# hellojialee/OffsetGuided

Measured on NVIDIA B200. Metric: decoded images/s @640 long-edge, higher is better.
Workload: dtype f32

## Files before the change

include/og_decoder.h:

```cpp
#ifndef OG_DECODER_H_
#define OG_DECODER_H_

#include <stdint.h>

#ifdef __cplusplus
extern "C" {
#endif

#define OG_ABI_VERSION 2
#define OG_MAX_IN_FLIGHT 16
#define OG_LIMB_COLS 13
#define OG_POSE_COLS 6
#define OG_MAX_KEYPOINTS 64
#define OG_MAX_LIMBS 64
#define OG_MAX_TOPK 128
#define OG_DTYPE_F32 0
#define OG_DTYPE_BF16 1
#define OG_DTYPE_F16 2

typedef enum og_status {
    OG_OK = 0,
    OG_ERR_INVALID_ARGUMENT = 1,
    OG_ERR_CUDA = 2,
    OG_ERR_OUT_OF_MEMORY = 3,
// ... 129 lines not shown
int og_plan_launch(og_handle *h, int32_t plan_id, void *stream);

typedef struct og_result {
    const float *poses;
    const int32_t *offsets;
    const int32_t *counts;
    int32_t n_images;
    int32_t total_rows;
    int32_t n_keypoints;
    int32_t buffer_id;
    const float *coco_keypoints;
    const double *coco_scores;
    const int32_t *coco_images;
} og_result;
int og_fetch_result(og_handle *h, og_result *out);

int og_set_frames(og_handle *h, const double *frames_host, int n);
int og_fetch_poses(og_handle *h, const float **poses_host, const int32_t **offset_host,
                   const int32_t **count_host, int32_t *total_rows);
int og_pending(const og_handle *h);

int og_copy_intermediates(og_handle *h, int n, float *det_score_dev, int32_t *det_index_dev,
                          float *limbs_dev, void *stream);

int64_t og_launch_count(const og_handle *h);

int og_set_fused(og_handle *h, int enable);

int og_set_graph(og_handle *h, int enable);
int64_t og_graph_replay_count(const og_handle *h);
int64_t og_graph_build_count(const og_handle *h);

int og_debug_k3_profile(uint64_t *out16, int reset);
int64_t og_fused_redo_count(const og_handle *h);
int64_t og_k3_redo_count(const og_handle *h);

int og_set_zero_copy(og_handle *h, int enable);
int64_t og_zero_copy_count(const og_handle *h);

int og_enable_stage_timing(og_handle *h, int enable);
int og_last_stage_times_ms(og_handle *h, float *out6);

#ifdef __cplusplus
}
#endif
#endif
```

offsetguided_b200/_lib.py:

```python
import ctypes
import os

_PKG_DIR = os.path.dirname(os.path.abspath(__file__))
LIB_PATH = os.path.join(_PKG_DIR, 'libogdecoder.so')

OG_LIMB_COLS = 13
OG_POSE_COLS = 6
OG_MAX_TOPK = 128
OG_MAX_IN_FLIGHT = 16
OG_DTYPE_F32 = 0
OG_DTYPE_BF16 = 1
OG_DTYPE_F16 = 2

c_int32_p = ctypes.POINTER(ctypes.c_int32)
c_float_p = ctypes.POINTER(ctypes.c_float)


class OgConfig(ctypes.Structure):
    _fields_ = [
        ('n_keypoints', ctypes.c_int32),
        ('n_limbs', ctypes.c_int32),
        ('limb_from', c_int32_p),
        ('limb_to', c_int32_p),
        ('topk', ctypes.c_int32),
# ... 47 lines not shown
    'og_flip_fuse_f32': (_i, [_vp, _vp, _vp, c_int32_p, c_int32_p, c_int32_p, _i, _i, _i, _i, _vp, _vp, _vp]),
    'og_flip_average_f32': (_i, [_vp, c_int32_p, _i, _i, _i, _i, _i, _vp, _vp]),
    'og_flip_cat_offsets_f32': (_i, [_vp, c_int32_p, c_int32_p, _i, _i, _i, _i, _i, _vp, _vp]),
    'og_resize_f32': (_i, [_vp, _vp, _i, _i, _i, _i, _i, _vp]),
    'og_decode_maps': (_i, [_vp, _vp, _vp, _vp, _i, _i, _i, _vp]),
    'og_decode_maps_ex': (_i, [_vp, _vp, _vp, _vp, _vp, _i, _i, _i, _i, _i, _vp]),
    'og_decode_features_host': (_i, [_vp, _vp, _vp, _i, _i, _i, _i, _i, _i, _i,
                                     c_int32_p, c_int32_p, c_int32_p, _i, _vp]),
    'og_decode_features_dev': (_i, [_vp, _vp, _vp, _i, _i, _i, _i, _i, _i, _i,
                                    c_int32_p, c_int32_p, c_int32_p, _i, _vp]),
    'og_decode_features_dev_ex': (_i, [_vp, _vp, _vp, _i, ctypes.c_int64, ctypes.c_int64, _i, _i, _i, _i, _i,
                                       _i, _i, c_int32_p, c_int32_p, c_int32_p, _i, _vp]),
    'og_decode_features_dev_strided': (_i, [_vp, _vp, _vp, _i, _i64_p, _i64_p, _i, _i, _i, _i, _i, _i, _i,
                                            c_int32_p, c_int32_p, c_int32_p, _i, _vp]),
    'og_fetch_poses': (_i, [_vp, ctypes.POINTER(c_float_p), ctypes.POINTER(c_int32_p),
                            ctypes.POINTER(c_int32_p), ctypes.POINTER(ctypes.c_int32)]),
    'og_decode_features_heads_dev': (_i, [_vp, _vp, _vp, _vp, _vp, _i, _i, _i, _i, _i, _i, _i,
                                          _i, _i, c_int32_p, c_int32_p, c_int32_p, _i, _vp]),
    'og_plan_features': (_i, [_vp, _vp, _vp, _i, ctypes.c_int64, ctypes.c_int64, _i, _i, _i, _i, _i,
                              _i, _i, c_int32_p, c_int32_p, c_int32_p, _i, ctypes.POINTER(ctypes.c_int32)]),
    'og_plan_features_strided': (_i, [_vp, _vp, _vp, _i, _i64_p, _i64_p, _i, _i, _i, _i, _i, _i, _i,
                                      c_int32_p, c_int32_p, c_int32_p, _i, ctypes.POINTER(ctypes.c_int32)]),
    'og_plan_launch': (_i, [_vp, ctypes.c_int32, _vp]),
    'og_fetch_result': (_i, [_vp, ctypes.POINTER(OgResult)]),
    'og_set_frames': (_i, [_vp, ctypes.POINTER(ctypes.c_double), _i]),
    'og_pending': (_i, [_vp]),
    'og_copy_intermediates': (_i, [_vp, _i, _vp, _vp, _vp, _vp]),
    'og_launch_count': (ctypes.c_int64, [_vp]),
    'og_set_fused': (_i, [_vp, _i]),
    'og_set_graph': (_i, [_vp, _i]),
    'og_graph_replay_count': (ctypes.c_int64, [_vp]),
    'og_graph_build_count': (ctypes.c_int64, [_vp]),
    'og_debug_k3_profile': (_i, [ctypes.POINTER(ctypes.c_uint64), _i]),
    'og_fused_redo_count': (ctypes.c_int64, [_vp]),
    'og_k3_redo_count': (ctypes.c_int64, [_vp]),
    'og_set_zero_copy': (_i, [_vp, _i]),
    'og_zero_copy_count': (ctypes.c_int64, [_vp]),
    'og_enable_stage_timing': (_i, [_vp, _i]),
    'og_last_stage_times_ms': (_i, [_vp, c_float_p]),
}

_lib = None


def load():
    global _lib
    if _lib is not None:
        return _lib
    if not os.path.exists(LIB_PATH):
        raise OgError(
            f'{LIB_PATH} is missing: build it with `python -m offsetguided_b200.build` '
            '(or __graft_entry__.build()).  There is no CPU fallback.')
    lib = ctypes.CDLL(LIB_PATH)
    for name, (restype, argtypes) in SIGNATURES.items():
        fn = getattr(lib, name)
        fn.restype = restype
        fn.argtypes = argtypes
    if lib.og_abi_version() != 2:
        raise OgError(f'ABI version mismatch: library reports {lib.og_abi_version()}')
    _lib = lib
    return lib


def check(status):
    if status != 0:
        lib = load()
# ... 13 lines not shown
```

offsetguided_b200/csrc/og_api.cu:

```cuda
#include <math.h>
#include <stdlib.h>
#include <string.h>

#include <algorithm>
#include <new>
#include <vector>

#include "og_common.cuh"

namespace og {

static thread_local char g_error[1024] = "";

void set_error(const char *fmt, ...) {
    va_list ap;
    va_start(ap, fmt);
    vsnprintf(g_error, sizeof(g_error), fmt, ap);
    va_end(ap);
}

}

using namespace og;

// ... 1560 lines not shown
    return OG_OK;
}

int64_t og_zero_copy_count(const og_handle *h) { return h ? h->zero_copy_calls : 0; }

int og_set_frames(og_handle *h, const double *frames_host, int n) {
    OG_REQUIRE(h && n >= 0 && (n == 0 || frames_host), "og_set_frames: null pointer");
    for (int i = 0; i < n; ++i)
        OG_REQUIRE(frames_host[4 * i + 2] != 0.0 && frames_host[4 * i + 3] != 0.0,
                   "og_set_frames: image %d has a zero scale", i);
    if (n > h->staged_cap) {
        double *grown = static_cast<double *>(realloc(h->staged_frames, (size_t)(n + 8) * 4 * sizeof(double)));
        if (!grown) {
            set_error("host allocation failed");
            return OG_ERR_OUT_OF_MEMORY;
        }
        h->staged_frames = grown;
        h->staged_cap = n + 8;
    }
    if (n) memcpy(h->staged_frames, frames_host, (size_t)n * 4 * sizeof(double));
    h->staged_n = n;
    return OG_OK;
}

int og_set_graph(og_handle *h, int enable) {
    OG_REQUIRE(h, "og_set_graph: null handle");
    h->graph_enabled = enable != 0;
    return OG_OK;
}

int64_t og_graph_replay_count(const og_handle *h) { return h ? h->graph_replays : 0; }
int64_t og_graph_build_count(const og_handle *h) { return h ? h->graph_builds : 0; }

int og_debug_k3_profile(uint64_t *out16, int reset) {
    OG_REQUIRE(out16, "og_debug_k3_profile: null pointer");
    return read_k3_profile(reinterpret_cast<unsigned long long *>(out16), reset != 0);
}

int og_enable_stage_timing(og_handle *h, int enable) {
    OG_REQUIRE(h, "og_enable_stage_timing: null handle");
    OG_TRY(check_device(h));
    if (enable) {
        for (int i = 0; i < kSlots; ++i)
            for (int e = 0; e < kStageEvents; ++e)
                if (!h->slots[i].ev[e]) OG_CUDA_TRY(cudaEventCreate(&h->slots[i].ev[e]));
    }
    h->timing = enable != 0;
    return OG_OK;
}

int og_last_stage_times_ms(og_handle *h, float *out6) {
    OG_REQUIRE(h && out6, "og_last_stage_times_ms: null pointer");
    OG_REQUIRE(h->fetched_slot >= 0 && h->slots[h->fetched_slot].timed,
               "og_last_stage_times_ms: enable stage timing, decode and fetch first");
    ResultSlot *slot = &h->slots[h->fetched_slot];
    OG_CUDA_TRY(cudaEventSynchronize(slot->ev[kStageEvents - 1]));
    static const int first[6] = {0, 1, 3, 4, 5, 6};
    for (int i = 0; i < 6; ++i)
        OG_CUDA_TRY(cudaEventElapsedTime(&out6[i], slot->ev[first[i]], slot->ev[first[i] + 1]));
    return OG_OK;
}

}
```

offsetguided_b200/csrc/og_common.cuh:

```cuda
#pragma once

#include <cuda_bf16.h>
#include <cuda_fp16.h>
#include <cuda_runtime.h>
#include <stdint.h>
#include <stdio.h>
#include <stdarg.h>

#include "../../include/og_decoder.h"

namespace og {

void set_error(const char *fmt, ...);

#define OG_CUDA_TRY(expr)                                                          \
    do {                                                                           \
        cudaError_t err__ = (expr);                                                \
        if (err__ != cudaSuccess) {                                                \
            og::set_error("%s:%d: %s failed: %s", __FILE__, __LINE__, #expr,       \
                          cudaGetErrorString(err__));                              \
            return err__ == cudaErrorMemoryAllocation ? OG_ERR_OUT_OF_MEMORY       \
                                                       : OG_ERR_CUDA;              \
        }                                                                          \
    } while (0)

#define OG_REQUIRE(cond, ...)                                                      \
    do {                                                                           \
        if (!(cond)) {                                                             \
            og::set_error(__VA_ARGS__);                                            \
            return OG_ERR_INVALID_ARGUMENT;                                        \
        }                                                                          \
    } while (0)

#define OG_TRY(expr)                                                               \
    do {                                                                           \
        int st__ = (expr);                                                         \
        if (st__ != OG_OK) return st__;                                            \
    } while (0)

constexpr int kChainCarveoutPercent = 58;

#ifdef __CUDACC__
template <auto Kernel>
inline void prefer_chain_carveout() {
    static unsigned long long done = 0ull;
    int dev = 0;
    if (cudaGetDevice(&dev) != cudaSuccess || dev < 0 || dev >= 64) return;
    if ((done >> dev) & 1ull) return;
    if (cudaFuncSetAttribute(Kernel, cudaFuncAttributePreferredSharedMemoryCarveout, kChainCarveoutPercent) !=
        cudaSuccess)
        (void)cudaGetLastError();
    done |= 1ull << dev;
}
#endif

constexpr int kCandCap = 2048;

__device__ __forceinline__ uint32_t ordered_bits(float v) {
    uint32_t u = __float_as_uint(v);
    return (u & 0x80000000u) ? ~u : (u | 0x80000000u);
}
__device__ __forceinline__ float from_ordered_bits(uint32_t o) {
    uint32_t u = (o & 0x80000000u) ? (o & 0x7fffffffu) : ~o;
    return __uint_as_float(u);
}
__device__ __forceinline__ uint64_t make_key(float v, uint32_t idx) {
    return ((uint64_t)(~ordered_bits(v)) << 32) | idx;
}
__device__ __forceinline__ float key_value(uint64_t key) {
    return from_ordered_bits(~(uint32_t)(key >> 32));
}

struct SkeletonDev {
// ... 71 lines not shown
    HeadSource jitter_lr;
};

struct PrepOut {
    int32_t *prep;
    float4 *rec;
    int32_t *cnt;
    float dist_max;
    int use_scale;
    int32_t *clear_word;
};

int launch_limb_score(const float *det_score, const int32_t *det_index, const float *offs,
                      const OffsetSource *lowres, const FlipTablesDev *flips, const float *scales,
                      const LimbExtras *extras, int n, int c, int l, int k, int h, int w,
                      const SkeletonDev &sk, float thre_hmp, float min_len, float resize_factor,
                      float *out_limbs, const PrepOut *prep, cudaStream_t s);

struct ChannelPerm {
    int32_t src[128];
};
int launch_flip_average(const float *in2n, float *out, int n, int ch, int h, int w,
                        const ChannelPerm &perm, bool negate_even, cudaStream_t s);
int launch_flip_cat_offsets(const float *off2n, float *out, int n, int l, int h, int w,
                            const ChannelPerm &limb_flip, const ChannelPerm &reserved, cudaStream_t s);

bool fused_supported(int n, int c, int scale, int h, int w);
void fused_scratch(int n, int c, int h, int w, int scale, size_t *flag_bytes, size_t *list_ints);
int launch_fused_candidates(const MapView &hmp, const FlipTablesDev &flips, int n, int n_total, int c, int h, int w,
                            int scale, bool cubic, bool flip, float thre, uint32_t *cand_count,
                            uint64_t *cand_keys, uint8_t *block_flag, int32_t *block_list,
                            int32_t *n_active, float *nhwc_heat, int sm_count, bool clear_first,
                            cudaStream_t s, int64_t *launches);

int launch_fuse_planes(const MapView &hmp, const FlipTablesDev &flips, int n, int c, int h, int w, bool flip,
                       const int32_t *plane_list, int count, float *out, cudaStream_t s);

struct CocoOut {
    const double *frames;
    float *keypoints;
    double *scores;
    int32_t *images;
    int image0;
};

struct GroupLaunch {
    int n, c, l, k;
    SkeletonDev sk;
    float dist_max;
    int use_scale;
    double person_thre;
    int sort_dim;
    int warp_rows;
    float *slab;
    size_t slab_stride;
    int32_t *prep;
    float4 *rec;
    int32_t *cnt;
    int32_t *redo;
    CocoOut coco;
    int32_t *lazy_flag;
};
int read_k3_profile(unsigned long long *out16, bool reset);
size_t group_smem_bytes(const GroupLaunch &g);
size_t group_warp_smem_bytes(const GroupLaunch &g);
size_t group_prep_ints(const GroupLaunch &g);
// ... 20 lines not shown
```

offsetguided_b200/csrc/og_fused.cu:

```cuda
#include "og_common.cuh"
#include "og_interp.cuh"

#include <algorithm>

namespace og {

namespace {

#ifndef OG_K1F_MIN_CTAS
#define OG_K1F_MIN_CTAS 4
#endif
constexpr int kFusedThreads = 256;
constexpr int kScanThreads = 256;
constexpr int kBlockCellsH = 8;
constexpr int kSub = 4;
constexpr unsigned kFull = 0xffffffffu;

__device__ __forceinline__ float4 ldg_stream4(const float *p) {
    float4 v;
    asm volatile("ld.global.nc.L1::no_allocate.v4.f32 {%0, %1, %2, %3}, [%4];"
                 : "=f"(v.x), "=f"(v.y), "=f"(v.z), "=f"(v.w)
                 : "l"(p));
    return v;
}

__device__ __forceinline__ float4 load_cells4(const float *p) { return ldg_stream4(p); }
__device__ __forceinline__ float4 load_cells4(const __nv_bfloat16 *p) {
    unsigned lo, hi;
    asm volatile("ld.global.nc.L1::no_allocate.v2.u32 {%0, %1}, [%2];" : "=r"(lo), "=r"(hi) : "l"(p));
    return make_float4(__uint_as_float(lo << 16), __uint_as_float(lo & 0xffff0000u),
                       __uint_as_float(hi << 16), __uint_as_float(hi & 0xffff0000u));
}

__device__ __forceinline__ float4 load_cells4(const __half *p) {
    unsigned lo, hi;
    asm volatile("ld.global.nc.L1::no_allocate.v2.u32 {%0, %1}, [%2];" : "=r"(lo), "=r"(hi) : "l"(p));
    const float2 a = __half22float2(*reinterpret_cast<const __half2 *>(&lo));
    const float2 b = __half22float2(*reinterpret_cast<const __half2 *>(&hi));
    return make_float4(a.x, a.y, b.x, b.y);
}

__device__ __forceinline__ unsigned abs_bits(float v) { return __float_as_uint(fabsf(v)); }

template <typename T, bool kFlip, bool kVec>
__global__ void __launch_bounds__(kScanThreads)
amax_scan_kernel(const T *__restrict__ hmp, size_t img_stride, const FlipTablesDev ft,
                 int N, int C, int h, int w, int bw_shift, int halo, float limit,
                 uint8_t *__restrict__ block_flag, int plane0, int planes, int per_plane) {
    const unsigned idx = blockIdx.x * (unsigned)kScanThreads + threadIdx.x;
    const unsigned pl = idx / (unsigned)per_plane;
    if (pl >= (unsigned)planes) return;
    const int local = (int)(idx - pl * (unsigned)per_plane);
    const int sxs = (w + kSub - 1) / kSub;
    const int band = local / sxs, sx = local - band * sxs;
    const int y0 = band * 2 * kSub, x0 = sx * kSub;
    const int block_w = 1 << bw_shift;
    const int bxs = (w + block_w - 1) >> bw_shift, bys = (h + kBlockCellsH - 1) / kBlockCellsH;
    {
        const int plane = plane0 + (int)pl;
        const int n = plane / C, c = plane - n * C;
        const T *a = hmp + (size_t)n * img_stride + (size_t)c * h * w;
        const T *b = nullptr;
        if (kFlip) b = hmp + (size_t)(N + n) * img_stride + (size_t)ft.kp[c] * h * w;
        uint8_t *flags = block_flag + (size_t)plane * bys * bxs;
        auto flag_blocks = [&](int xa, int xb, int y) {
            const int bx_lo = max(xa - halo, 0) >> bw_shift, bx_hi = min((xb + halo) >> bw_shift, bxs - 1);
            const int by_lo = max(y - halo, 0) / kBlockCellsH, by_hi = min((y + halo) / kBlockCellsH, bys - 1);
            for (int by = by_lo; by <= by_hi; ++by)
                for (int bx = bx_lo; bx <= bx_hi; ++bx) flags[by * bxs + bx] = 1;
        };
        if (kVec) {
#pragma unroll 1
            for (int r0 = 0; r0 < 2 * kSub; r0 += kSub) {
                float4 va[kSub], vb[kSub];
#pragma unroll
                for (int r = 0; r < kSub; ++r) {
                    const int y = min(y0 + r0 + r, h - 1);
                    va[r] = load_cells4(a + (size_t)y * w + x0);
                    if (kFlip) vb[r] = load_cells4(b + (size_t)y * w + (w - kSub - x0));
                }
                auto fused_row = [&](int r) {
                    float4 f = va[r];
                    if (kFlip) {
                        f.x = __fmul_rn(__fadd_rn(f.x, vb[r].w), 0.5f);
                        f.y = __fmul_rn(__fadd_rn(f.y, vb[r].z), 0.5f);
                        f.z = __fmul_rn(__fadd_rn(f.z, vb[r].y), 0.5f);
                        f.w = __fmul_rn(__fadd_rn(f.w, vb[r].x), 0.5f);
                    }
                    return f;
                };
                unsigned hot = 0u;
#pragma unroll
                for (int r = 0; r < kSub; ++r) {
                    const float4 f = fused_row(r);
                    const unsigned q = max(max(abs_bits(f.x), abs_bits(f.y)), max(abs_bits(f.z), abs_bits(f.w)));
                    if (!(__uint_as_float(q) < limit) && y0 + r0 + r < h) hot |= 1u << r;
                }
                if (hot != 0u) {
#pragma unroll
                    for (int r = 0; r < kSub; ++r) {
                        if (!((hot >> r) & 1u)) continue;
                        const float4 f = fused_row(r);
                        const bool c0 = !(fabsf(f.x) < limit), c1 = !(fabsf(f.y) < limit), c2 = !(fabsf(f.z) < limit),
                                   c3 = !(fabsf(f.w) < limit);
                        const int first = c0 ? 0 : (c1 ? 1 : (c2 ? 2 : 3));
                        const int last = c3 ? 3 : (c2 ? 2 : (c1 ? 1 : 0));
                        flag_blocks(x0 + first, x0 + last, y0 + r0 + r);
                    }
                }
            }
        } else {
            for (int r = 0; r < 2 * kSub; ++r) {
                const int y = y0 + r;
                if (y >= h) break;
                for (int j = 0; j < kSub; ++j) {
                    const int x = x0 + j;
                    if (x >= w) break;
                    float v = load_cell(a + (size_t)y * w + x);
                    if (kFlip) v = __fmul_rn(__fadd_rn(v, load_cell(b + (size_t)y * w + (w - 1 - x))), 0.5f);
                    if (!(fabsf(v) < limit)) flag_blocks(x, x, y);
                }
            }
        }
    }
}

constexpr int kNhwcPixels = 32;
constexpr int kNhwcThreads = 256;

template <typename T, bool kFlip>
__global__ void __launch_bounds__(kNhwcThreads)
amax_scan_nhwc_kernel(const T *__restrict__ hmp, size_t img_stride, size_t pix_stride, const FlipTablesDev ft,
                      int N, int C, int h, int w, int bw_shift, int halo, float limit,
                      uint8_t *__restrict__ block_flag, float *__restrict__ out) {
    __shared__ float s_row[OG_MAX_KEYPOINTS][kNhwcPixels + 1];
    const int gxs = (w + kNhwcPixels - 1) / kNhwcPixels, bands = (h + kBlockCellsH - 1) / kBlockCellsH;
    const unsigned cta = blockIdx.x;
    const int gx = (int)(cta % (unsigned)gxs);
    const int band = (int)((cta / (unsigned)gxs) % (unsigned)bands);
    const int n = (int)(cta / ((unsigned)gxs * (unsigned)bands));
    const int x0 = gx * kNhwcPixels, y0 = band * kBlockCellsH;
    const int px_n = min(kNhwcPixels, w - x0), y_end = min(y0 + kBlockCellsH, h);
    const int block_w = 1 << bw_shift;
    const int bxs = (w + block_w - 1) >> bw_shift, bys = (h + kBlockCellsH - 1) / kBlockCellsH;
    const size_t hw = (size_t)h * w;
    const T *a = hmp + (size_t)n * img_stride;
    const T *b = kFlip ? hmp + (size_t)(N + n) * img_stride : nullptr;
    const int cells = px_n * C;
    for (int y = y0; y < y_end; ++y) {
        for (int i = threadIdx.x; i < cells; i += kNhwcThreads) {
            const int px = i / C, c = i - px * C;
            const int x = x0 + px;
            float v = load_cell(a + ((size_t)y * w + x) * pix_stride + c);
            if (kFlip)
// ... 220 lines not shown
            for (int p = 0; p < S; ++p) {
                const bool pass = (mask >> p) & 1u;
                if (!__any_sync(kFull, pass)) continue;
                const float vp = v[p], vc = v[p + 1], vn = v[p + 2];
                const float lp = __shfl_up_sync(kFull, vp, 1), lc = __shfl_up_sync(kFull, vc, 1),
                            ln = __shfl_up_sync(kFull, vn, 1);
                const float rp = __shfl_down_sync(kFull, vp, 1), rc = __shfl_down_sync(kFull, vc, 1),
                            rn = __shfl_down_sync(kFull, vn, 1);
                if (pass) {
                    const int Y = Y0 + q * S + p;
                    bool peak = true;
                    if (lane > 0) peak = peak && !(lp > vc) && !(lc > vc) && !(ln > vc);
                    if (lane < 31) peak = peak && !(rp > vc) && !(rc > vc) && !(rn > vc);
                    if (peak && ((lane == 0 && X0 > 0) || (lane == 31 && X + 1 < W))) {
                        const int Xn = lane == 0 ? X - 1 : X + 1;
                        for (int dy = -1; dy <= 1 && peak; ++dy) {
                            if (Y + dy < 0 || Y + dy >= H) continue;
                            peak = !(tile_value<S, kCubic, LW, HALO>(lo, cx0, cy0, Xn, Y + dy) > vc);
                        }
                    }
                    if (peak) {
                        const uint32_t pos = atomicAdd(&cand_count[plane], 1u);
                        if (pos < (uint32_t)kCandCap)
                            cand_keys[(size_t)plane * kCandCap + pos] =
                                make_key(vc + 0.0f, (uint32_t)(Y * W + X));
                    }
                }
            }
        }
    }
}

template <typename Kernel>
int resident_per_sm(Kernel kernel) {
    int per_sm = 1;
    if (cudaOccupancyMaxActiveBlocksPerMultiprocessor(&per_sm, kernel, kFusedThreads, 0) != cudaSuccess ||
        per_sm < 1)
        per_sm = 1;
    return per_sm;
}

constexpr int kCtaWaves = 4;

template <typename T, int S, bool kCubic, bool kFlip>
int launch_blocks_t(const T *hmp, size_t img_stride, int n_total, int h, int w, float thre,
                    const int4 *block_list, const int32_t *n_active, uint32_t *cand_count,
                    uint64_t *cand_keys, int sm_count, size_t blocks, cudaStream_t s) {
    auto kernel = fused_block_kernel<T, S, kCubic, kFlip>;
    static const int per_sm = resident_per_sm(kernel);
    const int grid = (int)std::min<size_t>((blocks + kFusedThreads / 32 - 1) / (kFusedThreads / 32),
                                           (size_t)sm_count * per_sm * kCtaWaves);
    prefer_chain_carveout<fused_block_kernel<T, S, kCubic, kFlip>>();
    kernel<<<grid, kFusedThreads, 0, s>>>(hmp, img_stride, n_total, h, w, thre, block_list, n_active,
                                          cand_count, cand_keys);
    OG_CUDA_TRY(cudaGetLastError());
    return OG_OK;
}

template <typename T, int S>
int launch_blocks_s(const T *hmp, size_t img_stride, int n_total, int h, int w, bool cubic, bool flip,
                    float thre, const int4 *block_list, const int32_t *n_active, uint32_t *cand_count,
                    uint64_t *cand_keys, int sm_count, size_t blocks, cudaStream_t s) {
    if (cubic)
        return flip ? launch_blocks_t<T, S, true, true>(hmp, img_stride, n_total, h, w, thre, block_list, n_active, cand_count, cand_keys, sm_count, blocks, s)
                    : launch_blocks_t<T, S, true, false>(hmp, img_stride, n_total, h, w, thre, block_list, n_active, cand_count, cand_keys, sm_count, blocks, s);
    return flip ? launch_blocks_t<T, S, false, true>(hmp, img_stride, n_total, h, w, thre, block_list, n_active, cand_count, cand_keys, sm_count, blocks, s)
                : launch_blocks_t<T, S, false, false>(hmp, img_stride, n_total, h, w, thre, block_list, n_active, cand_count, cand_keys, sm_count, blocks, s);
}

inline size_t block_count(int n, int c, int h, int w, int scale) {
    const int bw = 32 / scale;
    return (size_t)n * c * ((w + bw - 1) / bw) * ((h + kBlockCellsH - 1) / kBlockCellsH);
}

}

bool fused_supported(int n, int c, int scale, int h, int w) {
    if (!(scale == 2 || scale == 4 || scale == 8)) return false;
    return block_count(n, c, h, w, scale) < 0x1fffffffULL && h < 65536 * kBlockCellsH && w < 65536 &&
           (unsigned long long)h * scale * w * scale < 0xffffffffULL;
}

void fused_scratch(int n, int c, int h, int w, int scale, size_t *flag_bytes, size_t *list_ints) {
    *flag_bytes = block_count(n, c, h, w, scale);
    *list_ints = 4 * block_count(n, c, h, w, scale);
}

namespace {
inline int scan_bw_shift(int scale) { return scale == 2 ? 4 : (scale == 4 ? 3 : 2); }
inline int scan_halo(bool cubic) { return cubic ? 2 : 1; }
inline float scan_limit(float thre, bool cubic) { return thre / (cubic ? 1.95f : 1.001f); }

template <typename T>
int launch_scan_nhwc_t(const T *hmp, size_t img_stride, size_t pix_stride, const FlipTablesDev &kp_flip_dev, int n,
                       int n_total, int c, int h, int w, int scale, bool cubic, bool flip, float thre,
                       uint8_t *block_flag, float *out, cudaStream_t s) {
    const long long ctas = (long long)n * ((w + kNhwcPixels - 1) / kNhwcPixels) *
                           ((h + kBlockCellsH - 1) / kBlockCellsH);
    if (ctas > 0x7fffffffLL) {
        set_error("fused K1: %lld scan CTAs of channels-last maps exceed one launch", ctas);
        return OG_ERR_UNSUPPORTED;
    }
#define OG_SCAN_NHWC(FLIP)                                                                                      \
    (prefer_chain_carveout<amax_scan_nhwc_kernel<T, FLIP>>(),                                                    \
     amax_scan_nhwc_kernel<T, FLIP><<<(unsigned)ctas, kNhwcThreads, 0, s>>>(                                     \
         hmp, img_stride, pix_stride, kp_flip_dev, n_total, c, h, w, scan_bw_shift(scale), scan_halo(cubic),     \
         scan_limit(thre, cubic), block_flag, out))
    if (flip) OG_SCAN_NHWC(true); else OG_SCAN_NHWC(false);
#undef OG_SCAN_NHWC
    OG_CUDA_TRY(cudaGetLastError());
    return OG_OK;
}

template <typename T>
int launch_fused_t(const T *hmp, size_t img_stride, const FlipTablesDev &kp_flip_dev, int n, int n_total,
                   int c, int h, int w, int scale, bool cubic, bool flip, float thre,
                   uint32_t *cand_count, uint64_t *cand_keys, uint8_t *block_flag, int32_t *block_list,
                   int32_t *n_active, int sm_count, bool clear_first, bool scan, cudaStream_t s,
                   int64_t *launches) {
    if (clear_first) {
        OG_CUDA_TRY(cudaMemsetAsync(cand_count, 0, sizeof(uint32_t) * (size_t)n * c, s));
        OG_CUDA_TRY(cudaMemsetAsync(n_active, 0, sizeof(int32_t), s));
    }

    const int sxs = (w + kSub - 1) / kSub, bands = (h + 2 * kSub - 1) / (2 * kSub);
    const int per_plane = bands * sxs, planes = scan ? n * c : 0;
    const int planes_per_launch = std::max(1, (int)std::min<long long>(n * c, 0x7fffffffLL / per_plane - 1));
    const int block_w = 32 / scale, halo = scan_halo(cubic);
    const int bw_shift = scan_bw_shift(scale);
    const float limit = scan_limit(thre, cubic);
    const size_t vec_bytes = 4 * sizeof(T);
    const bool vec = (w % kSub) == 0 && (reinterpret_cast<uintptr_t>(hmp) % vec_bytes) == 0 &&
                     (img_stride * sizeof(T)) % vec_bytes == 0;
#define OG_SCAN(FLIP, VEC)                                                                                     \
    (prefer_chain_carveout<amax_scan_kernel<T, FLIP, VEC>>(),                                                  \
     amax_scan_kernel<T, FLIP, VEC><<<scan_grid, kScanThreads, 0, s>>>(hmp, img_stride, kp_flip_dev, n_total, c, h, \
                                                                      w, bw_shift, halo, limit, block_flag, p0, pn, \
                                                                      per_plane))
    for (int p0 = 0; p0 < planes; p0 += planes_per_launch) {
        const int pn = std::min(planes_per_launch, planes - p0);
        const unsigned scan_grid = (unsigned)(((long long)pn * per_plane + kScanThreads - 1) / kScanThreads);
        if (flip) {
            if (vec) OG_SCAN(true, true); else OG_SCAN(true, false);
        } else {
            if (vec) OG_SCAN(false, true); else OG_SCAN(false, false);
        }
    }
#undef OG_SCAN
    OG_CUDA_TRY(cudaGetLastError());

    const size_t blocks = block_count(n, c, h, w, scale);
    int4 *list4 = reinterpret_cast<int4 *>(block_list);
    prefer_chain_carveout<block_list_kernel>();
    block_list_kernel<<<(unsigned)((blocks + 255) / 256), 256, 0, s>>>(
        block_flag, kp_flip_dev, c, flip ? 1 : 0, (w + block_w - 1) / block_w,
        (h + kBlockCellsH - 1) / kBlockCellsH, (long long)blocks, list4, n_active);
    OG_CUDA_TRY(cudaGetLastError());

    int st;
    switch (scale) {
        case 2: st = launch_blocks_s<T, 2>(hmp, img_stride, n_total, h, w, cubic, flip, thre, list4, n_active, cand_count, cand_keys, sm_count, blocks, s); break;
        case 4: st = launch_blocks_s<T, 4>(hmp, img_stride, n_total, h, w, cubic, flip, thre, list4, n_active, cand_count, cand_keys, sm_count, blocks, s); break;
        default: st = launch_blocks_s<T, 8>(hmp, img_stride, n_total, h, w, cubic, flip, thre, list4, n_active, cand_count, cand_keys, sm_count, blocks, s); break;
    }
    if (st == OG_OK && launches) *launches += 3;
    return st;
}
}

int launch_fused_candidates(const MapView &hmp, const FlipTablesDev &kp_flip_dev, int n, int n_total, int c,
                            int h, int w, int scale, bool cubic, bool flip, float thre,
                            uint32_t *cand_count, uint64_t *cand_keys, uint8_t *block_flag,
                            int32_t *block_list, int32_t *n_active, float *nhwc_heat, int sm_count,
                            bool clear_first, cudaStream_t s, int64_t *launches) {
    if (n == 0) return OG_OK;
    if (!fused_supported(n, c, scale, h, w)) {
        set_error("fused K1: scale %d / %d x %d maps are outside the supported range", scale, h, w);
        return OG_ERR_UNSUPPORTED;
    }
    if (hmp.is_channels_last()) {
        if (clear_first) {
            OG_CUDA_TRY(cudaMemsetAsync(cand_count, 0, sizeof(uint32_t) * (size_t)n * c, s));
            OG_CUDA_TRY(cudaMemsetAsync(n_active, 0, sizeof(int32_t), s));
        }
        int st;
        if (hmp.dtype == OG_DTYPE_BF16)
            st = launch_scan_nhwc_t(static_cast<const __nv_bfloat16 *>(hmp.ptr), hmp.image_stride, hmp.pixel_stride,
                                    kp_flip_dev, n, n_total, c, h, w, scale, cubic, flip, thre, block_flag, nhwc_heat, s);
        else if (hmp.dtype == OG_DTYPE_F16)
            st = launch_scan_nhwc_t(static_cast<const __half *>(hmp.ptr), hmp.image_stride, hmp.pixel_stride,
                                    kp_flip_dev, n, n_total, c, h, w, scale, cubic, flip, thre, block_flag, nhwc_heat, s);
        else
            st = launch_scan_nhwc_t(static_cast<const float *>(hmp.ptr), hmp.image_stride, hmp.pixel_stride,
                                    kp_flip_dev, n, n_total, c, h, w, scale, cubic, flip, thre, block_flag, nhwc_heat, s);
        OG_TRY(st);
        return launch_fused_t(static_cast<const float *>(nhwc_heat), (size_t)c * h * w, kp_flip_dev, n, n, c, h, w,
                              scale, cubic, false, thre, cand_count, cand_keys, block_flag, block_list, n_active,
                              sm_count, false, false, s, launches);
    }
    if (hmp.dtype == OG_DTYPE_BF16)
        return launch_fused_t(static_cast<const __nv_bfloat16 *>(hmp.ptr), hmp.image_stride, kp_flip_dev, n,
                              n_total, c, h, w, scale, cubic, flip, thre, cand_count, cand_keys, block_flag,
                              block_list, n_active, sm_count, clear_first, true, s, launches);
    if (hmp.dtype == OG_DTYPE_F16)
        return launch_fused_t(static_cast<const __half *>(hmp.ptr), hmp.image_stride, kp_flip_dev, n,
                              n_total, c, h, w, scale, cubic, flip, thre, cand_count, cand_keys, block_flag,
                              block_list, n_active, sm_count, clear_first, true, s, launches);
    return launch_fused_t(static_cast<const float *>(hmp.ptr), hmp.image_stride, kp_flip_dev, n, n_total, c,
                          h, w, scale, cubic, flip, thre, cand_count, cand_keys, block_flag, block_list,
                          n_active, sm_count, clear_first, true, s, launches);
}

namespace {
template <typename T>
__global__ void fuse_planes_kernel(const T *__restrict__ hmp, size_t img_stride, size_t plane_stride,
                                   size_t pix_stride, const FlipTablesDev ft, int n,
                                   int C, int h, int w, int flip, const int32_t *__restrict__ plane_list,
                                   float *__restrict__ out) {
    const int plane = plane_list[blockIdx.y];
    const int img = plane / C, c = plane - img * C;
    const size_t hw = (size_t)h * w;
    const T *a = hmp + (size_t)img * img_stride + (size_t)c * plane_stride;
    const T *b = flip ? hmp + (size_t)(n + img) * img_stride + (size_t)ft.kp[c] * plane_stride : nullptr;
    float *o = out + (size_t)blockIdx.y * hw;
    for (size_t i = (size_t)blockIdx.x * blockDim.x + threadIdx.x; i < hw; i += (size_t)gridDim.x * blockDim.x) {
        float v = load_cell(a + i * pix_stride);
        if (flip) {
            const int y = (int)(i / w), x = (int)(i - (size_t)y * w);
            v = __fmul_rn(__fadd_rn(v, load_cell(b + ((size_t)y * w + (w - 1 - x)) * pix_stride)), 0.5f);
        }
        o[i] = v;
    }
}
}

int launch_fuse_planes(const MapView &hmp, const FlipTablesDev &flips, int n, int c, int h, int w, bool flip,
                       const int32_t *plane_list, int count, float *out, cudaStream_t s) {
    if (count == 0) return OG_OK;
    const size_t hw = (size_t)h * w;
    const dim3 grid((unsigned)std::min<size_t>((hw + 255) / 256, 64), (unsigned)count);
    if (hmp.dtype == OG_DTYPE_BF16)
        fuse_planes_kernel<<<grid, 256, 0, s>>>(static_cast<const __nv_bfloat16 *>(hmp.ptr), hmp.image_stride, hmp.plane_stride, hmp.pixel_stride, flips, n, c, h, w, flip ? 1 : 0, plane_list, out);
    else if (hmp.dtype == OG_DTYPE_F16)
// ... 9 lines not shown
```

Before: 674,300.

## Pipeline amax scan through cp.async shared-memory ring with persistent grid

Rewrites the vectorized amax scan kernel as a persistent one-CTA-per-SM loop. It streams heatmap rows into a 64 KB cp.async shared-memory ring so global loads overlap with threshold checks. The fused block kernel's grid is resized from a register and shared-memory budget that reserves room for a co-resident scan CTA, and the extra waves multiplier is dropped. A debug residency query is also added. The risk is that a scan grid capped at one CTA per SM, plus the smaller fused grid, may leave bandwidth unused or add tail imbalance.

After: 702,400, median of 6. +4.2%, better.

```diff
diff --git a/include/og_decoder.h b/include/og_decoder.h
--- a/include/og_decoder.h
+++ b/include/og_decoder.h
@@ -185,6 +185,7 @@
 int64_t og_graph_build_count(const og_handle *h);
 
 int og_debug_k3_profile(uint64_t *out16, int reset);
+int og_debug_k1f_residency(int32_t *out, int capacity_rows, int32_t *rows);
 int64_t og_fused_redo_count(const og_handle *h);
 int64_t og_k3_redo_count(const og_handle *h);
 
diff --git a/offsetguided_b200/_lib.py b/offsetguided_b200/_lib.py
--- a/offsetguided_b200/_lib.py
+++ b/offsetguided_b200/_lib.py
@@ -103,6 +103,7 @@
     'og_graph_replay_count': (ctypes.c_int64, [_vp]),
     'og_graph_build_count': (ctypes.c_int64, [_vp]),
     'og_debug_k3_profile': (_i, [ctypes.POINTER(ctypes.c_uint64), _i]),
+    'og_debug_k1f_residency': (_i, [c_int32_p, _i, c_int32_p]),
     'og_fused_redo_count': (ctypes.c_int64, [_vp]),
     'og_k3_redo_count': (ctypes.c_int64, [_vp]),
     'og_set_zero_copy': (_i, [_vp, _i]),
diff --git a/offsetguided_b200/csrc/og_api.cu b/offsetguided_b200/csrc/og_api.cu
--- a/offsetguided_b200/csrc/og_api.cu
+++ b/offsetguided_b200/csrc/og_api.cu
@@ -1616,6 +1616,11 @@
 int64_t og_graph_replay_count(const og_handle *h) { return h ? h->graph_replays : 0; }
 int64_t og_graph_build_count(const og_handle *h) { return h ? h->graph_builds : 0; }
 
+int og_debug_k1f_residency(int32_t *out, int capacity_rows, int32_t *rows) {
+    OG_REQUIRE(out && rows && capacity_rows >= 0, "og_debug_k1f_residency: null pointer or negative capacity");
+    return og::k1f_residency(out, capacity_rows, rows);
+}
+
 int og_debug_k3_profile(uint64_t *out16, int reset) {
     OG_REQUIRE(out16, "og_debug_k3_profile: null pointer");
     return read_k3_profile(reinterpret_cast<unsigned long long *>(out16), reset != 0);
diff --git a/offsetguided_b200/csrc/og_common.cuh b/offsetguided_b200/csrc/og_common.cuh
--- a/offsetguided_b200/csrc/og_common.cuh
+++ b/offsetguided_b200/csrc/og_common.cuh
@@ -38,7 +38,10 @@
         if (st__ != OG_OK) return st__;                                            \
     } while (0)
 
-constexpr int kChainCarveoutPercent = 58;
+#ifndef OG_CHAIN_CARVEOUT
+#define OG_CHAIN_CARVEOUT 58
+#endif
+constexpr int kChainCarveoutPercent = OG_CHAIN_CARVEOUT;
 
 #ifdef __CUDACC__
 template <auto Kernel>
@@ -176,6 +179,9 @@
                             uint64_t *cand_keys, uint8_t *block_flag, int32_t *block_list,
                             int32_t *n_active, float *nhwc_heat, int sm_count, bool clear_first,
                             cudaStream_t s, int64_t *launches);
+
+constexpr int kResidencyCols = 10;
+int k1f_residency(int32_t *out, int capacity_rows, int32_t *rows);
 
 int launch_fuse_planes(const MapView &hmp, const FlipTablesDev &flips, int n, int c, int h, int w, bool flip,
                        const int32_t *plane_list, int count, float *out, cudaStream_t s);
diff --git a/offsetguided_b200/csrc/og_fused.cu b/offsetguided_b200/csrc/og_fused.cu
--- a/offsetguided_b200/csrc/og_fused.cu
+++ b/offsetguided_b200/csrc/og_fused.cu
@@ -16,110 +16,186 @@
 constexpr int kSub = 4;
 constexpr unsigned kFull = 0xffffffffu;
 
-__device__ __forceinline__ float4 ldg_stream4(const float *p) {
-    float4 v;
-    asm volatile("ld.global.nc.L1::no_allocate.v4.f32 {%0, %1, %2, %3}, [%4];"
-                 : "=f"(v.x), "=f"(v.y), "=f"(v.z), "=f"(v.w)
-                 : "l"(p));
-    return v;
-}
-
-__device__ __forceinline__ float4 load_cells4(const float *p) { return ldg_stream4(p); }
-__device__ __forceinline__ float4 load_cells4(const __nv_bfloat16 *p) {
-    unsigned lo, hi;
-    asm volatile("ld.global.nc.L1::no_allocate.v2.u32 {%0, %1}, [%2];" : "=r"(lo), "=r"(hi) : "l"(p));
-    return make_float4(__uint_as_float(lo << 16), __uint_as_float(lo & 0xffff0000u),
-                       __uint_as_float(hi << 16), __uint_as_float(hi & 0xffff0000u));
-}
-
-__device__ __forceinline__ float4 load_cells4(const __half *p) {
-    unsigned lo, hi;
-    asm volatile("ld.global.nc.L1::no_allocate.v2.u32 {%0, %1}, [%2];" : "=r"(lo), "=r"(hi) : "l"(p));
-    const float2 a = __half22float2(*reinterpret_cast<const __half2 *>(&lo));
-    const float2 b = __half22float2(*reinterpret_cast<const __half2 *>(&hi));
+#ifndef OG_SCAN_RING_KB
+#define OG_SCAN_RING_KB 64
+#endif
+#ifndef OG_SCAN_ROWS
+#define OG_SCAN_ROWS 2
+#endif
+constexpr int kScanRingBytes = OG_SCAN_RING_KB * 1024;
+constexpr int kScanRows = OG_SCAN_ROWS;
+constexpr int kScanMinCtas = 4;
+
+template <typename T, bool kFlip>
+__host__ __device__ constexpr int scan_stages() {
+    return kScanRingBytes / (kScanThreads * kScanRows * (kFlip ? 2 : 1) * kSub * (int)sizeof(T));
+}
+
+template <typename T>
+__device__ __forceinline__ void cp_async_cells4(void *smem, const T *gmem) {
+    const unsigned s = (unsigned)__cvta_generic_to_shared(smem);
+    if constexpr (sizeof(T) == 4)
+        asm volatile("cp.async.cg.shared.global [%0], [%1], 16;" ::"r"(s), "l"(gmem) : "memory");
+    else
+        asm volatile("cp.async.ca.shared.global [%0], [%1], 8;" ::"r"(s), "l"(gmem) : "memory");
+}
+__device__ __forceinline__ void cp_async_commit() { asm volatile("cp.async.commit_group;" ::: "memory"); }
+template <int N>
+__device__ __forceinline__ void cp_async_wait() { asm volatile("cp.async.wait_group %0;" ::"n"(N) : "memory"); }
+
+__device__ __forceinline__ float4 smem_cells4(const float *p) { return *reinterpret_cast<const float4 *>(p); }
+__device__ __forceinline__ float4 smem_cells4(const __nv_bfloat16 *p) {
+    const uint2 u = *reinterpret_cast<const uint2 *>(p);
+    return make_float4(__uint_as_float(u.x << 16), __uint_as_float(u.x & 0xffff0000u),
+                       __uint_as_float(u.y << 16), __uint_as_float(u.y & 0xffff0000u));
+}
+__device__ __forceinline__ float4 smem_cells4(const __half *p) {
+    const uint2 u = *reinterpret_cast<const uint2 *>(p);
+    const float2 a = __half22float2(*reinterpret_cast<const __half2 *>(&u.x));
+    const float2 b = __half22float2(*reinterpret_cast<const __half2 *>(&u.y));
     return make_float4(a.x, a.y, b.x, b.y);
 }
 
 __device__ __forceinline__ unsigned abs_bits(float v) { return __float_as_uint(fabsf(v)); }
 
 template <typename T, bool kFlip, bool kVec>
-__global__ void __launch_bounds__(kScanThreads)
+__global__ void __launch_bounds__(kScanThreads, kVec ? kScanMinCtas : 0)
 amax_scan_kernel(const T *__restrict__ hmp, size_t img_stride, const FlipTablesDev ft,
                  int N, int C, int h, int w, int bw_shift, int halo, float limit,
                  uint8_t *__restrict__ block_flag, int plane0, int planes, int per_plane) {
-    const unsigned idx = blockIdx.x * (unsigned)kScanThreads + threadIdx.x;
-    const unsigned pl = idx / (unsigned)per_plane;
-    if (pl >= (unsigned)planes) return;
-    const int local = (int)(idx - pl * (unsigned)per_plane);
     const int sxs = (w + kSub - 1) / kSub;
-    const int band = local / sxs, sx = local - band * sxs;
-    const int y0 = band * 2 * kSub, x0 = sx * kSub;
     const int block_w = 1 << bw_shift;
     const int bxs = (w + block_w - 1) >> bw_shift, bys = (h + kBlockCellsH - 1) / kBlockCellsH;
-    {
+    auto unit = [&](unsigned u, const T *&a, const T *&b, uint8_t *&flags, int &y0, int &x0) {
+        const unsigned pl = u / (unsigned)per_plane;
+        const int local = (int)(u - pl * (unsigned)per_plane);
+        const int band = local / sxs, sx = local - band * sxs;
+        y0 = band * 2 * kSub;
+        x0 = sx * kSub;
+        const int plane = plane0 + (int)pl;
+        const int n = plane / C, c = plane - n * C;
+        a = hmp + (size_t)n * img_stride + (size_t)c * h * w;
+        b = nullptr;
+        if (kFlip) b = hmp + (size_t)(N + n) * img_stride + (size_t)ft.kp[c] * h * w;
+        flags = block_flag + (size_t)plane * bys * bxs;
+    };
+    auto flag_blocks = [&](uint8_t *flags, int xa, int xb, int y) {
+        const int bx_lo = max(xa - halo, 0) >> bw_shift, bx_hi = min((xb + halo) >> bw_shift, bxs - 1);
+        const int by_lo = max(y - halo, 0) / kBlockCellsH, by_hi = min((y + halo) / kBlockCellsH, bys - 1);
+        for (int by = by_lo; by <= by_hi; ++by)
+            for (int bx = bx_lo; bx <= bx_hi; ++bx) flags[by * bxs + bx] = 1;
+    };
+    if constexpr (kVec) {
+        constexpr int kMaps = kFlip ? 2 : 1;
+        constexpr int kStages = scan_stages<T, kFlip>();
+        constexpr int kStagesPerUnit = 2 * kSub / kScanRows;
+        static_assert(kStages >= 2, "a ring of at least two slots");
+        extern __shared__ __align__(16) unsigned char s_ring_bytes[];
+        T(*ring)[kScanThreads][kSub] = reinterpret_cast<T(*)[kScanThreads][kSub]>(s_ring_bytes);
+        const int t = threadIdx.x;
+        const unsigned total = (unsigned)planes * (unsigned)per_plane;
+        const unsigned step = gridDim.x * (unsigned)kScanThreads;
+        const unsigned first = blockIdx.x * (unsigned)kScanThreads + t;
+        const int stages = first < total ? (int)((total - first + step - 1) / step) * kStagesPerUnit : 0;
+
+        const T *pa = nullptr, *pb = nullptr;
+        int py0 = 0;
+        int issued = 0, pslot = 0;
+        auto issue = [&]() {
+            if (issued < stages) {
+                const int j = issued % kStagesPerUnit;
+                if (j == 0) {
+                    uint8_t *unused;
+                    int x0;
+                    unit(first + (unsigned)(issued / kStagesPerUnit) * step, pa, pb, unused, py0, x0);
+                    pa += (size_t)py0 * w + x0;
+                    if (kFlip) pb += (size_t)py0 * w + (w - kSub - x0);
+                }
+                const int slot = pslot;
+                pslot = pslot + 1 == kStages ? 0 : pslot + 1;
+#pragma unroll
+                for (int r = 0; r < kScanRows; ++r) {
+                    const int dy = j * kScanRows + r;
+                    if (py0 + dy < h) {
+                        cp_async_cells4(ring[(slot * kScanRows + r) * kMaps][t], pa + (size_t)dy * w);
+                        if (kFlip) cp_async_cells4(ring[(slot * kScanRows + r) * kMaps + 1][t], pb + (size_t)dy * w);
+                    }
+                }
+            }
+            ++issued;
+            cp_async_commit();
+        };
+#pragma unroll
+        for (int k = 0; k < kStages - 1; ++k) issue();
+
+        const T *a, *b;
+        uint8_t *flags = nullptr;
+        int y0 = 0, x0 = 0, slot = 0;
+#pragma unroll 1
+        for (int k = 0; k < stages; ++k, slot = slot + 1 == kStages ? 0 : slot + 1) {
+            const int j = k % kStagesPerUnit;
+            if (j == 0) unit(first + (unsigned)(k / kStagesPerUnit) * step, a, b, flags, y0, x0);
+            cp_async_wait<kStages - 2>();
+            float4 va[kScanRows], vb[kScanRows];
+#pragma unroll
+            for (int r = 0; r < kScanRows; ++r) {
+                va[r] = smem_cells4(ring[(slot * kScanRows + r) * kMaps][t]);
+                if (kFlip) vb[r] = smem_cells4(ring[(slot * kScanRows + r) * kMaps + 1][t]);
+            }
+            issue();
+            auto fused_row = [&](int r) {
+                float4 f = va[r];
+                if (kFlip) {
+                    f.x = __fmul_rn(__fadd_rn(f.x, vb[r].w), 0.5f);
+                    f.y = __fmul_rn(__fadd_rn(f.y, vb[r].z), 0.5f);
+                    f.z = __fmul_rn(__fadd_rn(f.z, vb[r].y), 0.5f);
+                    f.w = __fmul_rn(__fadd_rn(f.w, vb[r].x), 0.5f);
+                }
+                return f;
+            };
+            const int yk = y0 + j * kScanRows;
+            unsigned hot = 0u;
+#pragma unroll
+            for (int r = 0; r < kScanRows; ++r) {
+                const float4 f = fused_row(r);
+                const unsigned q = max(max(abs_bits(f.x), abs_bits(f.y)), max(abs_bits(f.z), abs_bits(f.w)));
+                if (!(__uint_as_float(q) < limit) && yk + r < h) hot |= 1u << r;
+            }
+            if (hot != 0u) {
+#pragma unroll
+                for (int r = 0; r < kScanRows; ++r) {
+                    if (!((hot >> r) & 1u)) continue;
+                    const float4 f = fused_row(r);
+                    const bool c0 = !(fabsf(f.x) < limit), c1 = !(fabsf(f.y) < limit), c2 = !(fabsf(f.z) < limit),
+                               c3 = !(fabsf(f.w) < limit);
+                    const int first_c = c0 ? 0 : (c1 ? 1 : (c2 ? 2 : 3));
+                    const int last_c = c3 ? 3 : (c2 ? 2 : (c1 ? 1 : 0));
+                    flag_blocks(flags, x0 + first_c, x0 + last_c, yk + r);
+                }
+            }
+        }
+    } else {
+        const unsigned idx = blockIdx.x * (unsigned)kScanThreads + threadIdx.x;
+        const unsigned pl = idx / (unsigned)per_plane;
+        if (pl >= (unsigned)planes) return;
+        const int local = (int)(idx - pl * (unsigned)per_plane);
+        const int band = local / sxs, sx = local - band * sxs;
+        const int y0 = band * 2 * kSub, x0 = sx * kSub;
         const int plane = plane0 + (int)pl;
         const int n = plane / C, c = plane - n * C;
         const T *a = hmp + (size_t)n * img_stride + (size_t)c * h * w;
         const T *b = nullptr;
         if (kFlip) b = hmp + (size_t)(N + n) * img_stride + (size_t)ft.kp[c] * h * w;
         uint8_t *flags = block_flag + (size_t)plane * bys * bxs;
-        auto flag_blocks = [&](int xa, int xb, int y) {
-            const int bx_lo = max(xa - halo, 0) >> bw_shift, bx_hi = min((xb + halo) >> bw_shift, bxs - 1);
-            const int by_lo = max(y - halo, 0) / kBlockCellsH, by_hi = min((y + halo) / kBlockCellsH, bys - 1);
-            for (int by = by_lo; by <= by_hi; ++by)
-                for (int bx = bx_lo; bx <= bx_hi; ++bx) flags[by * bxs + bx] = 1;
-        };
-        if (kVec) {
-#pragma unroll 1
-            for (int r0 = 0; r0 < 2 * kSub; r0 += kSub) {
-                float4 va[kSub], vb[kSub];
-#pragma unroll
-                for (int r = 0; r < kSub; ++r) {
-                    const int y = min(y0 + r0 + r, h - 1);
-                    va[r] = load_cells4(a + (size_t)y * w + x0);
-                    if (kFlip) vb[r] = load_cells4(b + (size_t)y * w + (w - kSub - x0));
-                }
-                auto fused_row = [&](int r) {
-                    float4 f = va[r];
-                    if (kFlip) {
-                        f.x = __fmul_rn(__fadd_rn(f.x, vb[r].w), 0.5f);
-                        f.y = __fmul_rn(__fadd_rn(f.y, vb[r].z), 0.5f);
-                        f.z = __fmul_rn(__fadd_rn(f.z, vb[r].y), 0.5f);
-                        f.w = __fmul_rn(__fadd_rn(f.w, vb[r].x), 0.5f);
-                    }
-                    return f;
-                };
-                unsigned hot = 0u;
-#pragma unroll
-                for (int r = 0; r < kSub; ++r) {
-                    const float4 f = fused_row(r);
-                    const unsigned q = max(max(abs_bits(f.x), abs_bits(f.y)), max(abs_bits(f.z), abs_bits(f.w)));
-                    if (!(__uint_as_float(q) < limit) && y0 + r0 + r < h) hot |= 1u << r;
-                }
-                if (hot != 0u) {
-#pragma unroll
-                    for (int r = 0; r < kSub; ++r) {
-                        if (!((hot >> r) & 1u)) continue;
-                        const float4 f = fused_row(r);
-                        const bool c0 = !(fabsf(f.x) < limit), c1 = !(fabsf(f.y) < limit), c2 = !(fabsf(f.z) < limit),
-                                   c3 = !(fabsf(f.w) < limit);
-                        const int first = c0 ? 0 : (c1 ? 1 : (c2 ? 2 : 3));
-                        const int last = c3 ? 3 : (c2 ? 2 : (c1 ? 1 : 0));
-                        flag_blocks(x0 + first, x0 + last, y0 + r0 + r);
-                    }
-                }
-            }
-        } else {
-            for (int r = 0; r < 2 * kSub; ++r) {
-                const int y = y0 + r;
-                if (y >= h) break;
-                for (int j = 0; j < kSub; ++j) {
-                    const int x = x0 + j;
-                    if (x >= w) break;
-                    float v = load_cell(a + (size_t)y * w + x);
-                    if (kFlip) v = __fmul_rn(__fadd_rn(v, load_cell(b + (size_t)y * w + (w - 1 - x))), 0.5f);
-                    if (!(fabsf(v) < limit)) flag_blocks(x, x, y);
-                }
+        for (int r = 0; r < 2 * kSub; ++r) {
+            const int y = y0 + r;
+            if (y >= h) break;
+            for (int j = 0; j < kSub; ++j) {
+                const int x = x0 + j;
+                if (x >= w) break;
+                float v = load_cell(a + (size_t)y * w + x);
+                if (kFlip) v = __fmul_rn(__fadd_rn(v, load_cell(b + (size_t)y * w + (w - 1 - x))), 0.5f);
+                if (!(fabsf(v) < limit)) flag_blocks(flags, x, x, y);
             }
         }
     }
@@ -406,24 +482,33 @@
 }
 
 template <typename Kernel>
-int resident_per_sm(Kernel kernel) {
-    int per_sm = 1;
-    if (cudaOccupancyMaxActiveBlocksPerMultiprocessor(&per_sm, kernel, kFusedThreads, 0) != cudaSuccess ||
-        per_sm < 1)
-        per_sm = 1;
-    return per_sm;
-}
-
-constexpr int kCtaWaves = 4;
+int blocks_per_sm(Kernel kernel) {
+    int dev = 0, regs_sm = 65536, smem_sm = 0, per_sm = 1;
+    cudaFuncAttributes fa{};
+    if (cudaGetDevice(&dev) != cudaSuccess ||
+        cudaDeviceGetAttribute(&regs_sm, cudaDevAttrMaxRegistersPerMultiprocessor, dev) != cudaSuccess ||
+        cudaDeviceGetAttribute(&smem_sm, cudaDevAttrMaxSharedMemoryPerMultiprocessor, dev) != cudaSuccess ||
+        cudaFuncGetAttributes(&fa, kernel) != cudaSuccess ||
+        cudaOccupancyMaxActiveBlocksPerMultiprocessor(&per_sm, kernel, kFusedThreads, 0) != cudaSuccess) {
+        (void)cudaGetLastError();
+        return 1;
+    }
+    const int carveout = smem_sm / 100 * kChainCarveoutPercent;
+    const int reserved = 1024;
+    const int regs_cta = kFusedThreads * ((fa.numRegs + 7) & ~7);
+    const int by_regs = (regs_sm - kScanThreads * (65536 / (kScanMinCtas * kScanThreads))) / regs_cta;
+    const int by_smem = (carveout - kScanRingBytes - reserved) / ((int)fa.sharedSizeBytes + reserved);
+    return std::max(1, std::min(per_sm, std::min(by_regs, by_smem)));
+}
 
 template <typename T, int S, bool kCubic, bool kFlip>
 int launch_blocks_t(const T *hmp, size_t img_stride, int n_total, int h, int w, float thre,
                     const int4 *block_list, const int32_t *n_active, uint32_t *cand_count,
                     uint64_t *cand_keys, int sm_count, size_t blocks, cudaStream_t s) {
     auto kernel = fused_block_kernel<T, S, kCubic, kFlip>;
-    static const int per_sm = resident_per_sm(kernel);
+    static const int per_sm = blocks_per_sm(kernel);
     const int grid = (int)std::min<size_t>((blocks + kFusedThreads / 32 - 1) / (kFusedThreads / 32),
-                                           (size_t)sm_count * per_sm * kCtaWaves);
+                                           (size_t)sm_count * per_sm);
     prefer_chain_carveout<fused_block_kernel<T, S, kCubic, kFlip>>();
     kernel<<<grid, kFusedThreads, 0, s>>>(hmp, img_stride, n_total, h, w, thre, block_list, n_active,
                                           cand_count, cand_keys);
@@ -465,6 +550,18 @@
 inline int scan_halo(bool cubic) { return cubic ? 2 : 1; }
 inline float scan_limit(float thre, bool cubic) { return thre / (cubic ? 1.95f : 1.001f); }
 
+template <auto Kernel>
+void prefer_scan_ring() {
+    static unsigned long long done = 0ull;
+    int dev = 0;
+    if (cudaGetDevice(&dev) != cudaSuccess || dev < 0 || dev >= 64) return;
+    if ((done >> dev) & 1ull) return;
+    prefer_chain_carveout<Kernel>();
+    if (cudaFuncSetAttribute(Kernel, cudaFuncAttributeMaxDynamicSharedMemorySize, kScanRingBytes) != cudaSuccess)
+        return;
+    done |= 1ull << dev;
+}
+
 template <typename T>
 int launch_scan_nhwc_t(const T *hmp, size_t img_stride, size_t pix_stride, const FlipTablesDev &kp_flip_dev, int n,
                        int n_total, int c, int h, int w, int scale, bool cubic, bool flip, float thre,
@@ -499,28 +596,35 @@
 
     const int sxs = (w + kSub - 1) / kSub, bands = (h + 2 * kSub - 1) / (2 * kSub);
     const int per_plane = bands * sxs, planes = scan ? n * c : 0;
-    const int planes_per_launch = std::max(1, (int)std::min<long long>(n * c, 0x7fffffffLL / per_plane - 1));
     const int block_w = 32 / scale, halo = scan_halo(cubic);
     const int bw_shift = scan_bw_shift(scale);
     const float limit = scan_limit(thre, cubic);
     const size_t vec_bytes = 4 * sizeof(T);
     const bool vec = (w % kSub) == 0 && (reinterpret_cast<uintptr_t>(hmp) % vec_bytes) == 0 &&
                      (img_stride * sizeof(T)) % vec_bytes == 0;
-#define OG_SCAN(FLIP, VEC)                                                                                     \
-    (prefer_chain_carveout<amax_scan_kernel<T, FLIP, VEC>>(),                                                  \
-     amax_scan_kernel<T, FLIP, VEC><<<scan_grid, kScanThreads, 0, s>>>(hmp, img_stride, kp_flip_dev, n_total, c, h, \
-                                                                      w, bw_shift, halo, limit, block_flag, p0, pn, \
-                                                                      per_plane))
-    for (int p0 = 0; p0 < planes; p0 += planes_per_launch) {
-        const int pn = std::min(planes_per_launch, planes - p0);
-        const unsigned scan_grid = (unsigned)(((long long)pn * per_plane + kScanThreads - 1) / kScanThreads);
-        if (flip) {
-            if (vec) OG_SCAN(true, true); else OG_SCAN(true, false);
-        } else {
-            if (vec) OG_SCAN(false, true); else OG_SCAN(false, false);
-        }
-    }
+    if (planes > 0 && vec) {
+        const long long units = (long long)planes * per_plane;
+        const unsigned scan_grid = (unsigned)std::min<long long>(sm_count, (units + kScanThreads - 1) / kScanThreads);
+#define OG_SCAN_VEC(FLIP)                                                                                      \
+    (prefer_scan_ring<amax_scan_kernel<T, FLIP, true>>(),                                                      \
+     amax_scan_kernel<T, FLIP, true><<<scan_grid, kScanThreads, kScanRingBytes, s>>>(                          \
+         hmp, img_stride, kp_flip_dev, n_total, c, h, w, bw_shift, halo, limit, block_flag, 0, planes, per_plane))
+        if (flip) OG_SCAN_VEC(true); else OG_SCAN_VEC(false);
+#undef OG_SCAN_VEC
+    } else if (planes > 0) {
+        const int planes_per_launch = std::max(1, (int)std::min<long long>(n * c, 0x7fffffffLL / per_plane - 1));
+#define OG_SCAN(FLIP)                                                                                          \
+    (prefer_chain_carveout<amax_scan_kernel<T, FLIP, false>>(),                                                \
+     amax_scan_kernel<T, FLIP, false><<<scan_grid, kScanThreads, 0, s>>>(hmp, img_stride, kp_flip_dev, n_total, c, h, \
+                                                                       w, bw_shift, halo, limit, block_flag, p0, pn, \
+                                                                       per_plane))
+        for (int p0 = 0; p0 < planes; p0 += planes_per_launch) {
+            const int pn = std::min(planes_per_launch, planes - p0);
+            const unsigned scan_grid = (unsigned)(((long long)pn * per_plane + kScanThreads - 1) / kScanThreads);
+            if (flip) OG_SCAN(true); else OG_SCAN(false);
+        }
 #undef OG_SCAN
+    }
     OG_CUDA_TRY(cudaGetLastError());
 
     const size_t blocks = block_count(n, c, h, w, scale);
@@ -583,6 +687,54 @@
     return launch_fused_t(static_cast<const float *>(hmp.ptr), hmp.image_stride, kp_flip_dev, n, n_total, c,
                           h, w, scale, cubic, flip, thre, cand_count, cand_keys, block_flag, block_list,
                           n_active, sm_count, clear_first, true, s, launches);
+}
+
+namespace {
+struct ResidencyRows {
+    int32_t *out;
+    int capacity, count;
+};
+
+template <typename Kernel>
+int residency_row(ResidencyRows &r, Kernel kernel, int kind, int dtype, int s, int cubic, int flip, int dyn_smem,
+                  int per_sm) {
+    cudaFuncAttributes fa{};
+    OG_CUDA_TRY(cudaFuncGetAttributes(&fa, kernel));
+    const int32_t row[kResidencyCols] = {kind, dtype, s, cubic, flip, kind == 0 ? kScanThreads : kFusedThreads,
+                                         fa.numRegs, (int32_t)fa.sharedSizeBytes, dyn_smem, per_sm};
+    if (r.count < r.capacity)
+        for (int i = 0; i < kResidencyCols; ++i) r.out[(size_t)r.count * kResidencyCols + i] = row[i];
+    ++r.count;
+    return OG_OK;
+}
+
+template <typename T, int S>
+int residency_blocks(ResidencyRows &r, int dtype) {
+#define OG_ROW(CUBIC, FLIP)                                                                                  \
+    OG_TRY(residency_row(r, fused_block_kernel<T, S, CUBIC, FLIP>, 1, dtype, S, CUBIC, FLIP, 0,         \
+                         blocks_per_sm(fused_block_kernel<T, S, CUBIC, FLIP>)))
+    OG_ROW(false, false); OG_ROW(false, true); OG_ROW(true, false); OG_ROW(true, true);
+#undef OG_ROW
+    return OG_OK;
+}
+
+template <typename T>
+int residency_t(ResidencyRows &r, int dtype) {
+    OG_TRY(residency_row(r, amax_scan_kernel<T, false, true>, 0, dtype, 0, 0, 0, kScanRingBytes, 1));
+    OG_TRY(residency_row(r, amax_scan_kernel<T, true, true>, 0, dtype, 0, 0, 1, kScanRingBytes, 1));
+    OG_TRY((residency_blocks<T, 2>(r, dtype)));
+    OG_TRY((residency_blocks<T, 4>(r, dtype)));
+    return residency_blocks<T, 8>(r, dtype);
+}
+}
+
+int k1f_residency(int32_t *out, int capacity_rows, int32_t *rows) {
+    ResidencyRows r{out, capacity_rows, 0};
+    OG_TRY(residency_t<float>(r, OG_DTYPE_F32));
+    OG_TRY(residency_t<__nv_bfloat16>(r, OG_DTYPE_BF16));
+    OG_TRY(residency_t<__half>(r, OG_DTYPE_F16));
+    *rows = r.count;
+    return OG_OK;
 }
 
 namespace {
```
